# AberHu/TF-NAS

Hardware: AMD Instinct MI355X
Metric: supernet search images/sec (w-step + alpha-step) (higher is better)
Workload: dtype fp32

## Files before the change

tf-nas_amd/csrc/conv_kernels.hip:

```cpp
#include <stdlib.h>
#include "gemm_core.h"
#include "gemm_x3.h"
#include "kernels.h"
#include "prof.h"

constexpr int conv_lb(int mm) { return mm == 0 ? 4 : 3; }
constexpr int conv_wgrad_lb(int nt) { return nt >= 3 ? 3 : 4; }

template <int NT, int MM>
__global__ __launch_bounds__(256, conv_lb(MM)) void k_conv_fwd(TfnasCellDesc d, const float* __restrict__ x,
                                                               float* __restrict__ D, float* __restrict__ part,
                                                               const float* __restrict__ wf) {
    using T = GT<NT>;
    static_assert(T::B_ITERS == 1, "one B item per thread: its K position is the same in every chunk");
    __shared__ __attribute__((aligned(16))) float lds[T::LDS_FLOATS];
    const int BX = blockIdx.x, n0 = blockIdx.y * T::BN;
    const int mc = d.g[0].mc, mcp = d.g[0].mcp, off = d.g[0].off, M = d.M;
    const int H = d.H, W = d.W, Wo = d.Wo, HWo = d.Ho * d.Wo, S = d.stride, ic = d.ic;
    const int Po = d.N * HWo, K = 9 * ic;
    const int nrt = (Po + 127) >> 7, nchunks = (K + 15) >> 4;
    const int tid = threadIdx.x, lane = tid & 63, lr = lane & 15, lk = lane >> 4, wrow = (tid >> 6) * 32;

    float cs[NT], cq[NT];
#pragma unroll
    for (int j = 0; j < NT; ++j) cs[j] = cq[j] = 0.f;

    for (int rt = BX; rt < nrt; rt += gridDim.x) {
        f32x4 acc[2][NT];
        acc_zero<NT>(acc);
        int hi0[2], wi0[2];
        bool rok[2];
        const float* img[2];
#pragma unroll
        for (int i = 0; i < 2; ++i) {
            const int p = rt * 128 + wrow + 16 * i + lr, pc = min(p, Po - 1);
            const int n = pc / HWo, r = pc - n * HWo, ho = r / Wo, wo = r - ho * Wo;
            rok[i] = p < Po;
            hi0[i] = ho * S - 1;
            wi0[i] = wo * S - 1;
            img[i] = x + (size_t)n * H * W * ic;
        }
        int a_ky = 0, a_kx = 0, a_ch = 0;
        bool a_ok = false;
        auto pre = [&](int c) {
            const int ka = c * 16 + 4 * lk;
            a_ok = ka < K;
            const int ta = a_ok ? ka / ic : 0;
            a_ch = a_ok ? ka - ta * ic : 0;
            a_ky = ta / 3;
            a_kx = ta - 3 * a_ky;
        };
        auto tap_ok = [&](int i) -> bool {
            const int hi = hi0[i] + a_ky, wi = wi0[i] + a_kx;
            return a_ok && (unsigned)hi < (unsigned)H && (unsigned)wi < (unsigned)W;
        };
        auto la = [&](int c, int i, int kl) -> f32x4 {
            const int hi = hi0[i] + a_ky, wi = wi0[i] + a_kx;
            const size_t a = tap_ok(i) ? ((size_t)hi * W + wi) * ic + a_ch : 0;
            return ld4(img[i] + a);
        };
        auto xa = [&](f32x4 r, int c, int i, int kl) -> f32x4 { return (rok[i] && tap_ok(i)) ? r : zero4(); };
        auto lb = [&](int c, int n, int kl) -> f32x4 {
            return ld4(wf + (size_t)min(n0 + n, mc - 1) * K + min(c * 16 + kl, K - 4));
        };
        auto xb = [&](f32x4 r, int c, int n, int kl) -> f32x4 { return (c * 16 + kl < K && n0 + n < mc) ? r : zero4(); };
        gemm_adirect<NT, true, MM>(pre, la, xa, lb, xb, nchunks, acc, lds);
        emit_tile_rows<NT>(acc, lds, [&](int lrow, int lc, f32x4 v) {
            const int p = rt * 128 + lrow;
            if (p < Po && n0 + lc < mcp) st4_nt(D + ((size_t)p * M + off + n0 + lc), v);
        });
        acc_colstats<NT>(acc, cs, cq);
    }
    flush_colstats<NT>(cs, cq, lds, part + (size_t)BX * 2 * M + 2 * (size_t)off, n0, mcp);
}

template <int ACT>
__global__ __launch_bounds__(256) void k_conv_dd(TfnasCellDesc d, const float* __restrict__ dZ, const float* __restrict__ D,
                                                 const float* __restrict__ gate, const float* __restrict__ dpooled,
                                                 const double* __restrict__ stats2, const double* __restrict__ red2,
                                                 float* __restrict__ dd) {
    __shared__ f32x4 cst2[64];
    const int mc = d.g[0].mc, mcp = d.g[0].mcp, off = d.g[0].off, M = d.M;
    const int HWo = d.Ho * d.Wo, Po = d.N * HWo, c0 = blockIdx.y * 64;
    const int tid = threadIdx.x, q = tid & 15, ch = c0 + 4 * q;
    fill_cst2(cst2, d, 64, c0, mc, off, stats2, red2);
    __syncthreads();
    if (ch >= mcp) return;
    const bool has_se = d.g[0].se > 0;
    const float inv_hw = 1.f / (float)HWo;
    for (int p = blockIdx.x * 16 + (tid >> 4); p < Po; p += gridDim.x * 16) {
        const size_t a = (size_t)p * M + off + ch;
        const f32x4 dz = ld4_nt(dZ + a), dv = ld4_nt(D + a);
        f32x4 g4 = zero4(), dp4 = zero4();
        if (has_se) {
            const size_t t = (size_t)(p / HWo) * M + off + ch;
            g4 = ld4(gate + t);
            dp4 = ld4(dpooled + t) * splat4(inv_hw);
        }
        f32x4 r = bn2_dd<ACT>(cst2, 4 * q, dz, dv, has_se, g4, dp4);
#pragma unroll
        for (int j = 0; j < 4; ++j)
            if (ch + j >= mc) r[j] = 0.f;
        st4(dd + a, r);
    }
}

struct RawTap { f32x4 v; bool ok; };
template <int NT>
__global__ __launch_bounds__(256, conv_wgrad_lb(NT)) void k_conv_wgrad(TfnasCellDesc d, const float* __restrict__ dd,
                                                                       const float* __restrict__ x, int rows_per_split,
                                                                       float* __restrict__ part, size_t out_size) {
    using T = GT<NT>;
    __shared__ __attribute__((aligned(16))) float lds[T::LDS_FLOATS];
    const int ic = d.ic, mc = d.g[0].mc, mcp = d.g[0].mcp, off = d.g[0].off, M = d.M;
    const int H = d.H, W = d.W, Wo = d.Wo, HWo = d.Ho * d.Wo, S = d.stride, Po = d.N * HWo, NC = 9 * ic;
    float* __restrict__ gw = part + (size_t)blockIdx.x * out_size;
    const int m0 = blockIdx.y * 128, n0 = blockIdx.z * T::BN;
    const int r0 = blockIdx.x * rows_per_split, r1 = min(Po, r0 + rows_per_split);
    const int nchunks = (r1 - r0 + 15) >> 4;
    const int tid = threadIdx.x, lane = tid & 63, lr = lane & 15, lq = lane >> 4, wrow = (tid >> 6) * 32;
// ... 60 lines not shown
    const int W = d.W, HW = d.H * d.W, Ho = d.Ho, Wo = d.Wo, S = d.stride, ic = d.ic;
    const int P = d.N * HW, K = 9 * mcp;
    const int nrt = (P + 127) >> 7, nchunks = (K + 15) >> 4;
    const int tid = threadIdx.x, lane = tid & 63, lr = lane & 15, lk = lane >> 4, wrow = (tid >> 6) * 32;
    constexpr int BQ = T::BN / 4;
    const int bkl = tid / BQ, bcol = n0 + (tid % BQ) * 4;
    const bool bcok = tid < T::B_ITEMS && bcol < ic;
    const int bcc = min(bcol, ic - 4);

    for (int rt = blockIdx.x; rt < nrt; rt += gridDim.x) {
        f32x4 acc[2][NT];
        acc_zero<NT>(acc);
        int hi1[2], wi1[2];
        bool rok[2];
        const float* img[2];
#pragma unroll
        for (int i = 0; i < 2; ++i) {
            const int q = rt * 128 + wrow + 16 * i + lr, qc = min(q, P - 1);
            const int n = qc / HW, r = qc - n * HW, hi = r / W, wi = r - hi * W;
            rok[i] = q < P;
            hi1[i] = hi + 1;
            wi1[i] = wi + 1;
            img[i] = dd + (size_t)n * Ho * Wo * M + off;
        }
        int a_ky = 0, a_kx = 0, a_m = 0;
        bool a_ok = false;
        auto pre = [&](int c) {
            const int ka = c * 16 + 4 * lk;
            a_ok = ka < K;
            const int ta = a_ok ? ka / mcp : 0;
            a_m = a_ok ? ka - ta * mcp : 0;
            a_ky = ta / 3;
            a_kx = ta - 3 * a_ky;
        };
        auto src = [&](int i, int& ho, int& wo) -> bool {
            const int th = hi1[i] - a_ky, tw = wi1[i] - a_kx;
            ho = S == 2 ? th >> 1 : th;
            wo = S == 2 ? tw >> 1 : tw;
            const bool par = S == 1 || !((th | tw) & 1);
            return a_ok && par && th >= 0 && tw >= 0 && ho < Ho && wo < Wo;
        };
        auto la = [&](int c, int i, int kl) -> f32x4 {
            int ho, wo;
            const size_t a = src(i, ho, wo) ? ((size_t)ho * Wo + wo) * M + a_m : 0;
            return ld4(img[i] + a);
        };
        auto xa = [&](f32x4 r, int c, int i, int kl) -> f32x4 {
            int ho, wo;
            return (rok[i] && src(i, ho, wo)) ? r : zero4();
        };
        auto lb = [&](int c, int kl, int n) -> f32x4 { return ld4(wd + (size_t)min(c * 16 + bkl, K - 1) * ic + bcc); };
        auto xb = [&](f32x4 r, int c, int kl, int n) -> f32x4 { return (c * 16 + bkl < K && bcok) ? r : zero4(); };
        gemm_adirect<NT, false, MM>(pre, la, xa, lb, xb, nchunks, acc, lds);
        emit_tile_rows<NT>(acc, lds, [&](int lrow, int lc, f32x4 v) {
            const int q = rt * 128 + lrow;
            if (q < P && n0 + lc < ic) {
                const size_t a = (size_t)q * ic + n0 + lc;
                if (dres) v += ld4_nt(dres + a);
                st4_nt(dx + a, v);
            }
        });
    }
}

__global__ __launch_bounds__(256) void k_conv_repack(TfnasCellDesc d, float* __restrict__ wf, float* __restrict__ wd) {
    const int ic = d.ic, mc = d.g[0].mc, mcp = d.g[0].mcp;
    const float* __restrict__ w = d.g[0].w_expand;
    const int total = (wf ? mc : mcp) * 9 * ic;
    for (int idx = blockIdx.x * 256 + threadIdx.x; idx < total; idx += gridDim.x * 256) {
        if (wf) {
            const int m = idx / (9 * ic), k = idx - m * 9 * ic, tap = k / ic, c = k - tap * ic;
            wf[idx] = w[((size_t)m * ic + c) * 9 + tap];
        } else {
            const int kk = idx / ic, c = idx - kk * ic, tap = kk / mcp, m = kk - tap * mcp;
            wd[idx] = m < mc ? w[((size_t)m * ic + c) * 9 + tap] : 0.f;
        }
    }
}
static size_t conv_repack_floats(const TfnasCellDesc& d) { return ((size_t)9 * d.ic * d.g[0].mcp + 63) & ~(size_t)63; }

#define CONV_MM(mode, ...)                                     \
    switch (mode) {                                            \
        case 0: { constexpr int MM = 0; __VA_ARGS__; } break;  \
        case 1: { constexpr int MM = 1; __VA_ARGS__; } break;  \
        case 3: { constexpr int MM = 3; __VA_ARGS__; } break;  \
        default: { constexpr int MM = 6; __VA_ARGS__; } break; \
    }

static int conv_row_blocks(int rows, int col_tiles, size_t cap, int slots) {
    const int nrt = cdiv(rows, 128);
    int lim = nrt;
    if ((size_t)lim > cap) lim = (int)cap;
    if (lim > 1024) lim = 1024;
    if (lim < 1) lim = 1;
    long best_cost = -1;
    int best = 1;
    for (int gx = 1; gx <= lim; ++gx) {
        const long cost = (long)cdiv(gx * col_tiles, slots) * cdiv(nrt, gx);
        if (best_cost < 0 || cost <= best_cost) {
            best_cost = cost;
            best = gx;
        }
    }
    return best;
}

constexpr size_t CONV_MIN_STAT_ROWS = 128;
// ... 80 lines not shown
```

tf-nas_amd/csrc/gemm_core.h:

```cpp
#pragma once
#include "tfnas_dev.h"

template <int NT>
struct GT {
    static constexpr int BM = 128, BK = 16, BN = 16 * NT;
    static constexpr int LDA = BM + 16;
    static constexpr int LDB = (BN % 32 == 16) ? BN : BN + 16;
    static constexpr int A_FLOATS = BK * LDA, B_FLOATS = BK * LDB;
    static constexpr int X3_FLOATS = 1584 * NT;
    static constexpr int LDS_FLOATS = 2 * (A_FLOATS + B_FLOATS) > X3_FLOATS ? 2 * (A_FLOATS + B_FLOATS) : X3_FLOATS;
    static constexpr int B_ITEMS = BN * 4;
    static constexpr int B_ITERS = (B_ITEMS + 255) / 256;
};

template <int NT>
__device__ __forceinline__ void acc_zero(f32x4 (&acc)[2][NT]) {
#pragma unroll
    for (int i = 0; i < 2; ++i)
#pragma unroll
        for (int j = 0; j < NT; ++j) acc[i][j] = zero4();
}

struct XfId {
    __device__ __forceinline__ f32x4 operator()(f32x4 v, int, int, int, int) const { return v; }
// ... 107 lines not shown
    RB rb[T::B_ITERS];
    f32x4 cur[2];

#define TFNAS_B_IDX(i)                                                      \
    const int idx = tid + 256 * (i), b0_ = BKC ? (idx >> 2) : idx / (T::BN / 4), \
              b1_ = BKC ? (idx & 3) * 4 : (idx % (T::BN / 4)) * 4
#define TFNAS_GLOAD(c)                                                                      \
    {                                                                                       \
        pre(c);                                                                             \
        _Pragma("unroll") for (int i = 0; i < 2; ++i) ra[i] = la((c), i, 4 * lk);           \
        _Pragma("unroll") for (int i = 0; i < T::B_ITERS; ++i) {                            \
            TFNAS_B_IDX(i);                                                                 \
            if (idx < T::B_ITEMS) rb[i] = lb((c), b0_, b1_);                                \
        }                                                                                   \
    }
#define TFNAS_SSTORE(c, Bs)                                                                 \
    {                                                                                       \
        _Pragma("unroll") for (int i = 0; i < 2; ++i) cur[i] = xa(ra[i], (c), i, 4 * lk);   \
        _Pragma("unroll") for (int i = 0; i < T::B_ITERS; ++i) {                            \
            TFNAS_B_IDX(i);                                                                 \
            if (idx < T::B_ITEMS) {                                                         \
                const f32x4 v = xb(rb[i], (c), b0_, b1_);                                   \
                if (BKC) {                          \
                    const int r0_ = b1_ >> 2;                                               \
                    (Bs)[(r0_ + 0) * T::LDB + b0_] = v.x;                                   \
                    (Bs)[(r0_ + 4) * T::LDB + b0_] = v.y;                                   \
                    (Bs)[(r0_ + 8) * T::LDB + b0_] = v.z;                                   \
                    (Bs)[(r0_ + 12) * T::LDB + b0_] = v.w;                                  \
                } else {                                                                    \
                    st4(&(Bs)[((b0_ & 3) * 4 + (b0_ >> 2)) * T::LDB + b1_], v);             \
                }                                                                           \
            }                                                                               \
        }                                                                                   \
    }

    float* Bs0 = lds;
    float* Bs1 = lds + T::B_FLOATS;
    if (nchunks > 0) {
        TFNAS_GLOAD(0);
        TFNAS_SSTORE(0, Bs0);
    }
    __syncthreads();
    for (int c = 0; c < nchunks; ++c) {
        const float* Bs = (c & 1) ? Bs1 : Bs0;
        const bool more = (c + 1 < nchunks);
        if (more) TFNAS_GLOAD(c + 1);
#pragma unroll
        for (int ks = 0; ks < 4; ++ks) {
            const int k = ks * 4 + lk;
            const float a0 = cur[0][ks], a1 = cur[1][ks];
#pragma unroll
            for (int j = 0; j < NT; ++j) {
                const float b = Bs[k * T::LDB + 16 * j + lr];
                acc[0][j] = __builtin_amdgcn_mfma_f32_16x16x4f32(a0, b, acc[0][j], 0, 0, 0);
                acc[1][j] = __builtin_amdgcn_mfma_f32_16x16x4f32(a1, b, acc[1][j], 0, 0, 0);
            }
        }
        if (more) {
            if (c & 1) { TFNAS_SSTORE(c + 1, Bs0); } else { TFNAS_SSTORE(c + 1, Bs1); }
        }
        __syncthreads();
    }
#undef TFNAS_GLOAD
#undef TFNAS_SSTORE
#undef TFNAS_B_IDX
}

template <int NT, bool AK, bool BKC, class FA, class FB>
__device__ __forceinline__ void gemm_mainloop(FA& fa, FB& fb, int nchunks, f32x4 (&acc)[2][NT], float* lds) {
    auto la = [&](int c, int, int i0, int i1) -> f32x4 { return fa(c, i0, i1); };
    auto lb = [&](int c, int, int i0, int i1) -> f32x4 { return fb(c, i0, i1); };
    XfId id;
    gemm_mainloop2<NT, AK, BKC>(la, id, lb, id, nchunks, acc, lds);
}

template <int NT>
__device__ __forceinline__ void acc_colstats(const f32x4 (&acc)[2][NT], float (&s)[NT], float (&q)[NT]) {
#pragma unroll
    for (int j = 0; j < NT; ++j)
#pragma unroll
        for (int i = 0; i < 2; ++i) {
            const f32x4 v = acc[i][j];
            s[j] += (v.x + v.y) + (v.z + v.w);
            q[j] += (v.x * v.x + v.y * v.y) + (v.z * v.z + v.w * v.w);
        }
}

template <int NT>
__device__ __forceinline__ void flush_colstats(float (&s)[NT], float (&q)[NT], float* lds, float* part_row,
                                               int col0, int col_lim) {
    using T = GT<NT>;
    const int tid = threadIdx.x, lane = tid & 63, w = tid >> 6, lr = lane & 15;
#pragma unroll
    for (int j = 0; j < NT; ++j) {
        s[j] += __shfl_xor(s[j], 16, 64);
        s[j] += __shfl_xor(s[j], 32, 64);
        q[j] += __shfl_xor(q[j], 16, 64);
        q[j] += __shfl_xor(q[j], 32, 64);
    }
    if (lane < 16) {
#pragma unroll
        for (int j = 0; j < NT; ++j) {
            lds[(w * 2 + 0) * T::BN + 16 * j + lr] = s[j];
            lds[(w * 2 + 1) * T::BN + 16 * j + lr] = q[j];
        }
    }
    __syncthreads();
    if (tid < T::BN && col0 + tid < col_lim) {
        float ss = 0.f, qq = 0.f;
#pragma unroll
        for (int ww = 0; ww < 4; ++ww) {
            ss += lds[(ww * 2 + 0) * T::BN + tid];
            qq += lds[(ww * 2 + 1) * T::BN + tid];
        }
        part_row[2 * (size_t)(col0 + tid) + 0] = ss;
        part_row[2 * (size_t)(col0 + tid) + 1] = qq;
    }
    __syncthreads();
}

struct SlabNone {
    __device__ __forceinline__ void operator()(int, const float*) const {}
};
template <int NT, class FEmit, class FSlab = SlabNone>
__device__ __forceinline__ void emit_tile_rows(const f32x4 (&acc)[2][NT], float* lds, FEmit emit, FSlab slab = FSlab()) {
    using T = GT<NT>;
    constexpr int LDC = T::BN + 4, Q = T::BN / 4;
    static_assert(4 * 16 * LDC <= T::LDS_FLOATS, "C staging does not fit the GEMM LDS buffer");
    const int tid = threadIdx.x, lane = tid & 63, w = tid >> 6, lr = lane & 15, lq = lane >> 4;
    float* st = lds + w * 16 * LDC;
#pragma unroll
    for (int i = 0; i < 2; ++i) {
        __syncthreads();
#pragma unroll
        for (int j = 0; j < NT; ++j)
#pragma unroll
            for (int r = 0; r < 4; ++r) st[(4 * lq + r) * LDC + 16 * j + lr] = acc[i][j][r];
        __syncthreads();
#pragma unroll
        for (int it = 0; it < (16 * Q + 63) / 64; ++it) {
            const int idx = it * 64 + lane;
            if (idx < 16 * Q) {
                const int row = idx / Q, c4 = idx - row * Q;
                emit(w * 32 + 16 * i + row, 4 * c4, ld4(st + row * LDC + 4 * c4));
            }
        }
        slab(i, st);
    }
    __syncthreads();
}

static inline int pick_nt(int n, const int* cands, int ncand) {
    int best = cands[0];
    long best_pad = -1;
    for (int i = 0; i < ncand; ++i) {
        const int bn = 16 * cands[i];
        const long pad = (long)((n + bn - 1) / bn) * bn;
        if (best_pad < 0 || pad < best_pad || (pad == best_pad && cands[i] > best)) {
            best_pad = pad;
            best = cands[i];
        }
    }
    return best;
}
```

tf-nas_amd/csrc/gemm_kernels.hip:

```cpp
#include <stdlib.h>
#include <string.h>
#include "gemm_core.h"
#include "gemm_x3.h"
#include "kernels.h"
#include "prof.h"

__device__ __forceinline__ f32x4 stem_patch4(const float* __restrict__ img, const TfnasCellDesc& d, int p, int t0) {
    const int HW = d.H * d.W, n = p / HW, r = p - n * HW, ho = r / d.W, wo = r - ho * d.W;
    f32x4 v = zero4();
#pragma unroll
    for (int j = 0; j < 4; ++j) {
        const int t = t0 + j;
        if (t < 27) {
            const int ci = t / 9, rem = t - 9 * ci, ky = rem / 3, kx = rem - 3 * ky;
            const int hi = 2 * ho + ky - 1, wi = 2 * wo + kx - 1;
            if (hi >= 0 && hi < d.Hi && wi >= 0 && wi < d.Wi) v[j] = img[((size_t)(n * 3 + ci) * d.Hi + hi) * d.Wi + wi];
        }
    }
    return v;
}

constexpr int kLbBig = 3, kLbSmall = 4;
constexpr int kLbX3Big = 2, kLbX3Small = 3;
constexpr int gemm_lb(int nt, int mm) { return mm == 0 ? (nt >= 5 ? kLbBig : kLbSmall) : (nt >= 5 ? kLbX3Big : kLbX3Small); }
// ... 6 lines not shown
                                                    float* __restrict__ E, float* __restrict__ part) {
    using T = GT<NT>;
    __shared__ __attribute__((aligned(16))) float lds[T::LDS_FLOATS];
    const int L_ = blockIdx.x + gridDim.x * blockIdx.y;
    const bool ctf_ = d.G > 1;
    const int BX = ctf_ ? L_ / (int)gridDim.y : (int)blockIdx.x;
    int ty = ctf_ ? L_ % (int)gridDim.y : (int)blockIdx.y, g = 0;
    for (; g < d.G - 1; ++g) {
        const int t = (d.g[g].mcp + T::BN - 1) / T::BN;
        if (ty < t) break;
        ty -= t;
    }
    const int mc = d.g[g].mc, mcp = d.g[g].mcp, off = d.g[g].off;
    const float* __restrict__ w = d.g[g].w_expand;
    const int n0 = ty * T::BN;
    const int P = d.N * d.H * d.W, ic = d.ic, M = d.M;
    const int nrt = (P + 127) >> 7, nchunks = (ic + 15) >> 4;
    const int tid = threadIdx.x, lr = tid & 15, wrow = (tid >> 6) * 32;

    float cs[NT], cq[NT];
#pragma unroll
    for (int j = 0; j < NT; ++j) cs[j] = cq[j] = 0.f;

    for (int rt = BX; rt < nrt; rt += gridDim.x) {
        f32x4 acc[2][NT];
        acc_zero<NT>(acc);
        int prow[2];
        const float* arow[2];
#pragma unroll
        for (int i = 0; i < 2; ++i) {
            prow[i] = rt * 128 + wrow + 16 * i + lr;
            arow[i] = x + (size_t)min(prow[i], P - 1) * ic;
        }
        auto la = [&](int c, int i, int kl) -> f32x4 {
            const int k = c * 16 + kl;
            if (STEM) return (prow[i] < P && k < ic) ? stem_patch4(x, d, prow[i], k) : zero4();
            return ld4(arow[i] + min(k, ic - 4));
        };
        auto xa = [&](f32x4 r, int c, int i, int kl) -> f32x4 {
            if (STEM) return r;
            return (prow[i] < P && c * 16 + kl < ic) ? r : zero4();
        };
        auto lb = [&](int c, int n, int kl) -> f32x4 {
            const int col = n0 + n, k = c * 16 + kl;
            if (STEM) return (col < mc) ? ld4_guard(w + (size_t)col * ic, k, ic, false) : zero4();
            return ld4(w + (size_t)min(col, mc - 1) * ic + min(k, ic - 4));
        };
        auto xb = [&](f32x4 r, int c, int n, int kl) -> f32x4 {
            if (STEM) return r;
            return (n0 + n < mc && c * 16 + kl < ic) ? r : zero4();
        };
        PreNone pre;
        gemm_adirect<NT, true, MM>(pre, la, xa, lb, xb, nchunks, acc, lds);
        emit_tile_rows<NT>(acc, lds, [&](int lrow, int lc, f32x4 v) {
            const int p = rt * 128 + lrow;
            if (p < P && n0 + lc < mcp) st4_nt(E + ((size_t)p * M + off + n0 + lc), v);
        });
        acc_colstats<NT>(acc, cs, cq);
    }
    flush_colstats<NT>(cs, cq, lds, part + (size_t)BX * 2 * M + 2 * (size_t)off, n0, mcp);
}

template <int NT, int ACT, int MM>
__global__ __launch_bounds__(256, gemm_lb(NT, MM)) void k_project_fwd(TfnasCellDesc d, const float* __restrict__ D,
                                                     const float* __restrict__ gate,
                                                     const double* __restrict__ stats2, float* __restrict__ Pr,
                                                     float* __restrict__ part, int nsplit, float* __restrict__ prp) {
    using T = GT<NT>;
    extern __shared__ __attribute__((aligned(16))) float lds[];
    const int zr = blockIdx.z / nsplit, ks = blockIdx.z - zr * nsplit;
    int g = 0;
    for (int c = 0; c < d.G; ++c) {
        int rank = 0;
        for (int o = 0; o < d.G; ++o) rank += (d.g[o].mcp > d.g[c].mcp) || (d.g[o].mcp == d.g[c].mcp && o < c);
        if (rank == zr) g = c;
    }
    const int mc = d.g[g].mc, mcp = d.g[g].mcp, off = d.g[g].off;
    const bool has_se = d.g[g].se > 0, w_al = (mc & 3) == 0;
    const float* gbase = has_se ? gate : D;
    const size_t se01 = has_se ? 1 : 0;
    const float* __restrict__ w = d.g[g].w_proj;
    const int n0 = blockIdx.y * T::BN;
    const int HW = d.Ho * d.Wo, Po = d.N * HW, oc = d.oc, M = d.M;
    const int nrt = (Po + 127) >> 7, nchunks_all = (mcp + 15) >> 4;
    const int per = (nchunks_all + nsplit - 1) / nsplit, cb = ks * per;
    const int nchunks = max(0, min(nchunks_all, cb + per) - cb);
    float* __restrict__ dst = ks == 0 ? Pr : prp + (size_t)(ks - 1) * d.G * Po * oc;
    const int tid = threadIdx.x, lr = tid & 15, wrow = (tid >> 6) * 32;

    float2* cst = reinterpret_cast<float2*>(lds + T::LDS_FLOATS);
    for (int c = tid; c < ((mcp + 15) & ~15); c += 256)
        cst[c] = (c < mc) ? bn_consts(stats2 + 2 * (size_t)(off + c), 1.0 / (double)Po, d.eps) : make_float2(0.f, 0.f);
    __syncthreads();

    float cs[NT], cq[NT];
#pragma unroll
    for (int j = 0; j < NT; ++j) cs[j] = cq[j] = 0.f;

    for (int rt = blockIdx.x; rt < nrt; rt += gridDim.x) {
        f32x4 acc[2][NT];
        acc_zero<NT>(acc);
        size_t arow[2], grow[2];
        bool rok[2];
#pragma unroll
        for (int i = 0; i < 2; ++i) {
            const int p = rt * 128 + wrow + 16 * i + lr, pc = min(p, Po - 1);
            rok[i] = p < Po;
            arow[i] = (size_t)pc * M + off;
            grow[i] = ((size_t)(pc / HW) * M + off) * se01;
        }
        auto la = [&](int c, int i, int kl) -> Raw2 {
            const int k = min((cb + c) * 16 + kl, mcp - 4);
            Raw2 r;
            r.a = ld4(D + (arow[i] + k));
            r.b = ld4(gbase + grow[i] + k * se01);
            return r;
        };
        auto xa = [&](Raw2 r, int c, int i, int kl) -> f32x4 {
            const int k = (cb + c) * 16 + kl;
            f32x4 v = r.a;
            const int kc = min(k, mcp - 4);
            const float2 c0 = cst[kc], c1 = cst[kc + 1], c2 = cst[kc + 2], c3 = cst[kc + 3];
            v.x = act_f<ACT>((v.x - c0.x) * c0.y);
            v.y = act_f<ACT>((v.y - c1.x) * c1.y);
            v.z = act_f<ACT>((v.z - c2.x) * c2.y);
            v.w = act_f<ACT>((v.w - c3.x) * c3.y);
            if (has_se) v *= r.b;
            return (rok[i] && k < mcp) ? v : zero4();
        };
        auto lb = [&](int c, int n, int kl) -> f32x4 {
            const int o = n0 + n, k = (cb + c) * 16 + kl;
            if (MM == 0 && !w_al) return (o < oc) ? ld4_guard(w + (size_t)o * mc, k, mc, false) : zero4();
            return ld4(w + (size_t)min(o, oc - 1) * mc + min(k, mc - 4));
        };
        auto xb = [&](f32x4 r, int c, int n, int kl) -> f32x4 {
            if (MM == 0 && !w_al) return r;
            return (n0 + n < oc && (cb + c) * 16 + kl < mc) ? r : zero4();
        };
        PreNone pre;
        gemm_adirect<NT, true, MM>(pre, la, xa, lb, xb, nchunks, acc, lds);
        emit_tile_rows<NT>(acc, lds, [&](int lrow, int lc, f32x4 v) {
            const int p = rt * 128 + lrow;
            if (p < Po && n0 + lc < oc) st4(dst + ((size_t)g * Po + p) * oc + n0 + lc, v);
        });
        acc_colstats<NT>(acc, cs, cq);
    }
    if (nsplit == 1)
        flush_colstats<NT>(cs, cq, lds, part + (size_t)blockIdx.x * 2 * d.G * oc + 2 * (size_t)g * oc, n0, oc);
}

__global__ __launch_bounds__(256) void k_pr_reduce(float* __restrict__ Pr, const float* __restrict__ prp, int nz, int G,
                                                   int Po, int oc, int rps, float* __restrict__ part) {
    __shared__ f32x4 rs[256], rq[256];
    const int tid = threadIdx.x, ocq = oc >> 2, stride = (256 / ocq) * ocq;
    const int g = blockIdx.y;
    const int r0 = blockIdx.x * rps, r1 = min(Po, r0 + rps);
    const size_t base = ((size_t)g * Po + r0) * ocq, zs = (size_t)G * Po * ocq;
    f32x4* __restrict__ p4 = reinterpret_cast<f32x4*>(Pr) + base;
    const f32x4* __restrict__ z4 = reinterpret_cast<const f32x4*>(prp) + base;
    const int n4 = (r1 - r0) * ocq;
    f32x4 s = zero4(), q = zero4();
    if (tid < stride) {
        for (int i = tid; i < n4; i += stride) {
            f32x4 v = p4[i];
            for (int z = 0; z < nz; ++z) v += z4[(size_t)z * zs + i];
            p4[i] = v;
            s += v;
            q += v * v;
        }
    }
    rs[tid] = s;
    rq[tid] = q;
    __syncthreads();
    for (int c = tid; c < oc; c += 256) {
        const int cq = c >> 2, comp = c & 3;
        float ts = 0.f, tq = 0.f;
        for (int k = cq; k < stride; k += ocq) {
            ts += rs[k][comp];
            tq += rq[k][comp];
        }
        float* row = part + (size_t)blockIdx.x * 2 * G * oc + 2 * ((size_t)g * oc + c);
        row[0] = ts;
        row[1] = tq;
    }
}

struct Bn3Tab {
    float *mean, *rstd, *a3, *b3, *c3;
};
__device__ __forceinline__ Bn3Tab bn3_tab_fill(float* base, int ocp, const TfnasCellDesc& d, int g,
                                               const double* stats3, const double* red3, const float* wmix) {
    Bn3Tab t{base, base + ocp, base + 2 * ocp, base + 3 * ocp, base + 4 * ocp};
    const int Po = d.N * d.Ho * d.Wo;
    const double inv = 1.0 / (double)Po;
// ... 125 lines not shown
    constexpr int NC = (T::BN + 63) / 64;
    float2 c2f[NC];
    bool cokf[NC];
    const int HW = d.Ho * d.Wo;
    const bool has_se = d.g[g].se > 0;
    if (FOLD) {
#pragma unroll
        for (int c = 0; c < NC; ++c) {
            const int col = (tid & 63) + 64 * c;
            cokf[c] = col < T::BN && n0 + col < mcp;
            c2f[c] = (cokf[c] && n0 + col < mc) ? bn_consts(stats2 + 2 * (size_t)(off + n0 + col), 1.0 / (double)Po, d.eps)
                                               : make_float2(0.f, 0.f);
        }
    }
    __syncthreads();

    for (int rt = BX; rt < nrt; rt += gridDim.x) {
        f32x4 acc[2][NT];
        acc_zero<NT>(acc);
        const float* drow[2];
        const float* qrow[2];
        bool rok[2];
#pragma unroll
        for (int i = 0; i < 2; ++i) {
            const int p = rt * 128 + wrow + 16 * i + lr, pc = min(p, Po - 1);
            rok[i] = p < Po;
            drow[i] = dout + (size_t)pc * oc;
            qrow[i] = Pr + ((size_t)g * Po + pc) * oc;
        }
        auto la = [&](int c, int i, int kl) -> Raw2 {
            const int o = min(c * 16 + kl, oc - 4);
            Raw2 r;
            r.a = ld4(drow[i] + o);
            r.b = ld4(qrow[i] + o);
            return r;
        };
        auto xa = [&](Raw2 r, int c, int i, int kl) -> f32x4 {
            const int o = c * 16 + kl;
            const f32x4 v = bn3_fold_dp(tab, min(o, oc - 4), r.a, r.b);
            return (rok[i] && o < oc) ? v : zero4();
        };
        auto lb = [&](int c, int kl, int n) -> f32x4 {
            const int o = c * 16 + kl;
            if (MM == 0 && !w_al) return (o < oc) ? ld4_guard(w + (size_t)o * mc, n0 + n, mc, false) : zero4();
            return ld4(w + (size_t)min(o, oc - 1) * mc + min(n0 + n, mc - 4));
        };
        auto xb = [&](f32x4 r, int c, int kl, int n) -> f32x4 {
            if (MM == 0 && !w_al) return r;
            return (c * 16 + kl < oc && n0 + n < mc) ? r : zero4();
        };
        PreNone pre;
        gemm_adirect<NT, false, MM>(pre, la, xa, lb, xb, nchunks, acc, lds);
        if (!FOLD) {
            emit_tile_rows<NT>(acc, lds, [&](int lrow, int lc, f32x4 v) {
                const int p = rt * 128 + lrow;
                if (p < Po && n0 + lc < mcp) st4_nt(dZ + ((size_t)p * M + off + n0 + lc), v);
            });
        } else {
            constexpr int LDC = T::BN + 4;
            const int w = tid >> 6, lane = tid & 63;
            const int pw0 = rt * 128 + w * 32;
            const int imgA = min(pw0, Po - 1) / HW, bnd = (imgA + 1) * HW;
            float sum[2][FOLD_Q][NC];
#pragma unroll
            for (int a = 0; a < 2; ++a)
#pragma unroll
                for (int q = 0; q < FOLD_Q; ++q)
#pragma unroll
                    for (int c = 0; c < NC; ++c) sum[a][q][c] = 0.f;
            const float* Dcol = D + off + n0;
            emit_tile_rows<NT>(acc, lds,
                               [&](int lrow, int lc, f32x4 v) {
                                   const int p = rt * 128 + lrow;
                                   if (p < Po && n0 + lc < mcp) st4_nt(dZ + ((size_t)p * M + off + n0 + lc), v);
                               },
                               [&](int i, const float* st) {
                                   if (d.act == TFNAS_ACT_RELU)
                                       fold_slab<NT, TFNAS_ACT_RELU>(st, LDC, Dcol, M, pw0 + 16 * i, Po, bnd, c2f, cokf, has_se, sum);
                                   else
                                       fold_slab<NT, TFNAS_ACT_SWISH>(st, LDC, Dcol, M, pw0 + 16 * i, Po, bnd, c2f, cokf, has_se, sum);
                               });
            static_assert(4 * 2 * FOLD_Q * T::BN + 4 <= T::LDS_FLOATS, "fold staging does not fit the GEMM LDS buffer");
            float* comb = lds;
            int* meta = reinterpret_cast<int*>(lds + 4 * 2 * FOLD_Q * T::BN);
#pragma unroll
            for (int a = 0; a < 2; ++a)
#pragma unroll
                for (int q = 0; q < FOLD_Q; ++q)
#pragma unroll
                    for (int c = 0; c < NC; ++c)
                        if (lane + 64 * c < T::BN) comb[((w * 2 + a) * FOLD_Q + q) * T::BN + lane + 64 * c] = sum[a][q][c];
            if (lane == 0) meta[w] = imgA;
            __syncthreads();
            const int img0 = min(rt * 128, Po - 1) / HW, imgL = min(rt * 128 + 127, Po - 1) / HW;
            const int nq = has_se ? FOLD_Q : 2;
            for (int o = tid; o < FOLD_SLOTS * FOLD_Q * T::BN; o += 256) {
                const int sl = o / (FOLD_Q * T::BN), q = (o / T::BN) % FOLD_Q, col = o % T::BN;
                if (img0 + sl > imgL || q >= nq || n0 + col >= mcp) continue;
                float t = 0.f;
#pragma unroll
                for (int ww = 0; ww < 4; ++ww)
#pragma unroll
                    for (int a = 0; a < 2; ++a)
                        if (meta[ww] + a - img0 == sl) t += comb[((ww * 2 + a) * FOLD_Q + q) * T::BN + col];
                rec[(((size_t)rt * FOLD_SLOTS + sl) * FOLD_Q + q) * M + off + n0 + col] = t;
            }
            __syncthreads();
        }
    }
}

constexpr int wgrad_lb(int nt) { return nt >= 5 ? 2 : (nt >= 3 ? 3 : 4); }

template <int NT, int ACT>
__global__ __launch_bounds__(256, wgrad_lb(NT)) void k_project_wgrad(TfnasCellDesc d, const float* __restrict__ dout,
                                                       const float* __restrict__ Pr, const float* __restrict__ D,
                                                       const float* __restrict__ gate,
                                                       const double* __restrict__ stats2,
                                                       const double* __restrict__ stats3,
                                                       const double* __restrict__ red3,
                                                       const float* __restrict__ wmix, int rows_per_split,
                                                       int ntiles_o, float* __restrict__ part, size_t out_size) {
    using T = GT<NT>;
    extern __shared__ __attribute__((aligned(16))) float lds[];
    const int g = blockIdx.z / ntiles_o, n0 = (blockIdx.z % ntiles_o) * T::BN;
    const int mc = d.g[g].mc, mcp = d.g[g].mcp, off = d.g[g].off;
    const bool has_se = d.g[g].se > 0;
    const float* gbase = has_se ? gate : D;
    const size_t se01 = has_se ? 1 : 0;
    size_t poff = 0;
    for (int gg = 0; gg < g; ++gg) poff += (size_t)d.g[gg].mc * d.oc;
    float* __restrict__ gw = part + (size_t)blockIdx.x * out_size + poff;
    const int m0 = blockIdx.y * 128;
    if (m0 >= mcp) return;
// ... 148 lines not shown
        bool is_x;
        int k0, klim_a, klim_b, ld_a;
        size_t aoff;
        const float* bsrc;
        const float* ssrc;
        auto pre = [&](int c) {
            c += cbeg;
            if (c >= mchunks) {
                is_x = true;
                k0 = (c - mchunks) * 16;
                klim_a = klim_b = ld_a = ic;
                aoff = 0;
                bsrc = gram;
                ssrc = cb1 + 1;
                return;
            }
            int g = 0;
            for (; g < d.G - 1; ++g) {
                const int t = (d.g[g].mcp + 15) >> 4;
                if (c < t) break;
                c -= t;
            }
            is_x = false;
            k0 = c * 16;
            klim_a = d.g[g].mcp;
            klim_b = d.g[g].mc;
            ld_a = M;
            aoff = d.g[g].off;
            bsrc = d.g[g].w_expand;
            ssrc = cb1 + 4 * (size_t)d.g[g].off + 1;
        };
        int prow[2];
#pragma unroll
        for (int i = 0; i < 2; ++i) prow[i] = rt * 128 + wrow + 16 * i + lr;
        auto la = [&](int c, int i, int kl) -> f32x4 {
            const int pc = min(prow[i], P - 1), k = min(k0 + kl, klim_a - 4);
            return ld4((is_x ? x : dEh) + (size_t)pc * ld_a + aoff + k);
        };
        auto xa = [&](f32x4 r, int c, int i, int kl) -> f32x4 {
            return (prow[i] < P && k0 + kl < klim_a) ? r : zero4();
        };
        auto lb = [&](int c, int kl, int n) -> RawWS {
            const int kc = min(k0 + kl, klim_b - 1), col = min(n0 + n, ic - 4);
            RawWS r;
            r.w = ld4(bsrc + (size_t)kc * ic + col);
            r.s = ssrc[is_x ? 0 : 4 * (size_t)kc];
            return r;
        };
        auto xb = [&](RawWS r, int c, int kl, int n) -> f32x4 {
            const f32x4 v = is_x ? -r.w : splat4(r.s) * r.w;
            return (n0 + n < ic && k0 + kl < klim_b) ? v : zero4();
        };
        gemm_adirect<NT, false, MM>(pre, la, xa, lb, xb, nchunks, acc, lds);
        emit_tile_rows<NT>(acc, lds, [&](int lrow, int lc, f32x4 v) {
            const int p = rt * 128 + lrow, c = n0 + lc;
            if (p < P && c < ic) {
                if (plain) v += ld4(gram + (size_t)ic * ic + c);
                if (add_res) v += splat4(sumw) * ld4(dout + (size_t)p * d.oc + c);
                if (add_sink) v = sink_add(v, sink_w, ld4(add_src + (size_t)p * ic + c));
                st4(dst + (size_t)p * ic + c, v);
            }
        });
    }
}

__global__ __launch_bounds__(256) void k_dx_reduce(TfnasCellDesc d, const float* __restrict__ dxp, int nsplit,
                                                   const float* __restrict__ gram, const float* __restrict__ dout,
                                                   const float* __restrict__ wmix, float* __restrict__ dx,
                                                   const float* __restrict__ add_src,
                                                   const float* __restrict__ add_scale) {
    const float sink_w = add_src ? add_scale[0] : 0.f;
    const size_t n4 = (size_t)d.N * d.H * d.W * d.ic / 4;
    const int iq = d.ic / 4;
    const float* __restrict__ bias = gram + (size_t)d.ic * d.ic;
    float sumw = 1.f;
    if (wmix) {
        sumw = 0.f;
        for (int g = 0; g < d.G; ++g) sumw += wmix[g];
    }
    for (size_t i = (size_t)blockIdx.x * 256 + threadIdx.x; i < n4; i += (size_t)gridDim.x * 256) {
        f32x4 v = ld4(bias + 4 * (int)(i % iq));
        if (d.has_res) v += splat4(sumw) * ld4(dout + 4 * i);
        for (int z = 0; z < nsplit; ++z) v += ld4(dxp + (size_t)z * n4 * 4 + 4 * i);
        if (add_src) v = sink_add(v, sink_w, ld4(add_src + 4 * i));
        st4(dx + 4 * i, v);
    }
}

template <int NT>
__global__ __launch_bounds__(256) void k_expand_gram(TfnasCellDesc d, const float* __restrict__ cb1, int chunks_per_split,
                                                     int nsplit, float* __restrict__ part) {
    using T = GT<NT>;
    __shared__ __attribute__((aligned(16))) float lds[T::LDS_FLOATS];
    const int ic = d.ic;
    const int m0 = blockIdx.y * 128, n0 = blockIdx.z * T::BN;
    const int xs = (int)blockIdx.x;
    int mchunks = 0;
    for (int g = 0; g < d.G; ++g) mchunks += (d.g[g].mcp + 15) >> 4;
    const int cbeg = xs * chunks_per_split;
    const int nchunks = max(0, min(mchunks, cbeg + chunks_per_split) - cbeg);
    const f32x4* cb = reinterpret_cast<const f32x4*>(cb1);
    const int tid = threadIdx.x, lane = tid & 63, lr = lane & 15, lq = lane >> 4, wrow = (tid >> 6) * 32;
    float* __restrict__ out = part + (size_t)blockIdx.x * (size_t)(ic + 4) * ic;

    f32x4 acc[2][NT];
    acc_zero<NT>(acc);
    auto locate = [&](int c, int& g, int& k0) {
// ... 628 lines not shown
```

tf-nas_amd/csrc/gemm_x3.h:

```cpp
#pragma once
#include "gemm_core.h"

typedef __bf16 bf16x8 __attribute__((ext_vector_type(8)));
typedef unsigned u32x4 __attribute__((ext_vector_type(4)));
typedef unsigned u32x2 __attribute__((ext_vector_type(2)));

__device__ __forceinline__ unsigned x3_bits(float v) { return __builtin_bit_cast(unsigned, v); }
__device__ __forceinline__ float x3_float(unsigned v) { return __builtin_bit_cast(float, v); }
__device__ __forceinline__ unsigned x3_pack(unsigned a, unsigned b) { return __builtin_amdgcn_perm(b, a, 0x07060302u); }

struct X3Planes { u32x2 h, m, l; };
template <int TERMS>
__device__ __forceinline__ X3Planes x3_split4(f32x4 v) {
    unsigned hb[4], mb[4], lb[4];
#pragma unroll
    for (int e = 0; e < 4; ++e) {
        hb[e] = x3_bits(v[e]);
        mb[e] = lb[e] = 0;
        if (TERMS > 1) {
            const float r1 = v[e] - x3_float(hb[e] & 0xffff0000u);
            mb[e] = x3_bits(r1);
            if (TERMS > 3) lb[e] = x3_bits(r1 - x3_float(mb[e] & 0xffff0000u));
        }
    }
// ... 63 lines not shown
                                         : (b1 >> 4) * X::TS + (4 * h + (b0 >> 2)) * 128 + (b0 & 3) * 32 + ((b1 & 15) >> 2) * 8;
                *reinterpret_cast<u32x2*>(Bs + off) = p.h;
                if (TERMS > 1) *reinterpret_cast<u32x2*>(Bs + PLANE + off) = p.m;
                if (TERMS > 3) *reinterpret_cast<u32x2*>(Bs + 2 * PLANE + off) = p.l;
            }
        }
    };
    auto sstore = [&](int C, unsigned char* Bs) {
        X3Planes p0[2], p1[2];
        sstore_half(2 * C, 0, true, Bs, p0);
        sstore_half(2 * C + 1, 1, 2 * C + 1 < nchunks, Bs, p1);
#pragma unroll
        for (int i = 0; i < 2; ++i) {
            ca[i][0] = u32x4{p0[i].h.x, p0[i].h.y, p1[i].h.x, p1[i].h.y};
            ca[i][1] = u32x4{p0[i].m.x, p0[i].m.y, p1[i].m.x, p1[i].m.y};
            ca[i][2] = u32x4{p0[i].l.x, p0[i].l.y, p1[i].l.x, p1[i].l.y};
        }
    };
    const unsigned rd = BKC ? lr * 64 + ((lk ^ x3_fperm(lr >> 2)) * 16) : lk * 128 + lr * 8;
    auto frag = [&](const unsigned char* p, int j) -> bf16x8 {
        if (BKC) return __builtin_bit_cast(bf16x8, *reinterpret_cast<const u32x4*>(p + rd + j * 1024));
        typedef short s16x4 __attribute__((ext_vector_type(4)));
        typedef short s16x8 __attribute__((ext_vector_type(8)));
        typedef __attribute__((address_space(3))) s16x4* lds_p;
        const s16x4 a = __builtin_amdgcn_ds_read_tr16_b64_v4i16((lds_p)(p + rd + j * X::TS));
        const s16x4 b = __builtin_amdgcn_ds_read_tr16_b64_v4i16((lds_p)(p + rd + j * X::TS + 512));
        const s16x8 v = {a.x, a.y, a.z, a.w, b.x, b.y, b.z, b.w};
        return __builtin_bit_cast(bf16x8, v);
    };

    if (nC > 0) {
        gload(0);
        sstore(0, lds);
    }
    __syncthreads();
    for (int C = 0; C < nC; ++C) {
        const unsigned char* Bs = lds + (C & 1) * BUF;
        const bool more = C + 1 < nC;
        if (more) gload(C + 1);
        bf16x8 ah[2], am[2], al[2];
#pragma unroll
        for (int i = 0; i < 2; ++i) {
            ah[i] = __builtin_bit_cast(bf16x8, ca[i][0]);
            am[i] = __builtin_bit_cast(bf16x8, ca[i][1]);
            al[i] = __builtin_bit_cast(bf16x8, ca[i][2]);
        }
#pragma unroll
        for (int j = 0; j < NT; ++j) {
            const bf16x8 bh = frag(Bs, j);
            bf16x8 bm = bh, bl = bh;
            if (TERMS > 1) bm = frag(Bs + PLANE, j);
            if (TERMS > 3) bl = frag(Bs + 2 * PLANE, j);
#define TFNAS_X3_MF(a, b)                                                                   \
    acc[0][j] = __builtin_amdgcn_mfma_f32_16x16x32_bf16(a[0], b, acc[0][j], 0, 0, 0);       \
    acc[1][j] = __builtin_amdgcn_mfma_f32_16x16x32_bf16(a[1], b, acc[1][j], 0, 0, 0);
            if (TERMS > 3) { TFNAS_X3_MF(al, bh) TFNAS_X3_MF(am, bm) TFNAS_X3_MF(ah, bl) }
            if (TERMS > 1) { TFNAS_X3_MF(am, bh) TFNAS_X3_MF(ah, bm) }
            TFNAS_X3_MF(ah, bh)
#undef TFNAS_X3_MF
        }
        if (more) sstore(C + 1, lds + ((C + 1) & 1) * BUF);
        __syncthreads();
    }
}

template <int NT, bool BKC, int MM, class PRE, class LA, class XA, class LB, class XB>
__device__ __forceinline__ void gemm_adirect(PRE& pre, LA& la, XA& xa, LB& lb, XB& xb, int nchunks, f32x4 (&acc)[2][NT],
                                             float* lds) {
    if constexpr (MM == 0) gemm_mainloop_adirect<NT, BKC>(pre, la, xa, lb, xb, nchunks, acc, lds);
    else gemm_mainloop_adirect_x3<NT, BKC, MM>(pre, la, xa, lb, xb, nchunks, acc, lds);
}
```

Before: 3908.

## Swap MFMA operands to transpose accumulator layout and simplify epilogues

Swaps the A/B operands of the MFMA instructions so each lane holds four consecutive output columns of one row instead of four rows of one column. With this transposed accumulator layout, several GEMM epilogues store f32x4 results straight to global memory without LDS staging. The remaining staged paths use per-wave vector LDS writes with wave-level ordering instead of block-wide barriers, and column statistics are reduced with DPP row operations instead of cross-lane shuffles. This removes LDS round-trips and __syncthreads in the epilogue, but relies on the new lane-to-element mapping being applied consistently everywhere acc is consumed.

Measured after the change: 3882 (median of 2 runs). About the same (-0.6%).

```diff
diff --git a/tf-nas_amd/csrc/conv_kernels.hip b/tf-nas_amd/csrc/conv_kernels.hip
--- a/tf-nas_amd/csrc/conv_kernels.hip
+++ b/tf-nas_amd/csrc/conv_kernels.hip
@@ -65,7 +65,7 @@
         };
         auto xb = [&](f32x4 r, int c, int n, int kl) -> f32x4 { return (c * 16 + kl < K && n0 + n < mc) ? r : zero4(); };
         gemm_adirect<NT, true, MM>(pre, la, xa, lb, xb, nchunks, acc, lds);
-        emit_tile_rows<NT>(acc, lds, [&](int lrow, int lc, f32x4 v) {
+        emit_tile_staged<NT>(acc, lds, [&](int lrow, int lc, f32x4 v) {
             const int p = rt * 128 + lrow;
             if (p < Po && n0 + lc < mcp) st4_nt(D + ((size_t)p * M + off + n0 + lc), v);
         });
@@ -232,7 +232,7 @@
         auto lb = [&](int c, int kl, int n) -> f32x4 { return ld4(wd + (size_t)min(c * 16 + bkl, K - 1) * ic + bcc); };
         auto xb = [&](f32x4 r, int c, int kl, int n) -> f32x4 { return (c * 16 + bkl < K && bcok) ? r : zero4(); };
         gemm_adirect<NT, false, MM>(pre, la, xa, lb, xb, nchunks, acc, lds);
-        emit_tile_rows<NT>(acc, lds, [&](int lrow, int lc, f32x4 v) {
+        emit_tile_direct<NT>(acc, [&](int lrow, int lc, f32x4 v) {
             const int q = rt * 128 + lrow;
             if (q < P && n0 + lc < ic) {
                 const size_t a = (size_t)q * ic + n0 + lc;
diff --git a/tf-nas_amd/csrc/gemm_core.h b/tf-nas_amd/csrc/gemm_core.h
--- a/tf-nas_amd/csrc/gemm_core.h
+++ b/tf-nas_amd/csrc/gemm_core.h
@@ -183,8 +183,8 @@
 #pragma unroll
             for (int j = 0; j < NT; ++j) {
                 const float b = Bs[k * T::LDB + 16 * j + lr];
-                acc[0][j] = __builtin_amdgcn_mfma_f32_16x16x4f32(a0, b, acc[0][j], 0, 0, 0);
-                acc[1][j] = __builtin_amdgcn_mfma_f32_16x16x4f32(a1, b, acc[1][j], 0, 0, 0);
+                acc[0][j] = __builtin_amdgcn_mfma_f32_16x16x4f32(b, a0, acc[0][j], 0, 0, 0);
+                acc[1][j] = __builtin_amdgcn_mfma_f32_16x16x4f32(b, a1, acc[1][j], 0, 0, 0);
             }
         }
         if (more) {
@@ -205,35 +205,44 @@
     gemm_mainloop2<NT, AK, BKC>(la, id, lb, id, nchunks, acc, lds);
 }
 
+template <int CTRL>
+__device__ __forceinline__ float dpp_mov(float v) {
+    return __builtin_bit_cast(float, __builtin_amdgcn_update_dpp(0, __builtin_bit_cast(int, v), CTRL, 0xf, 0xf, false));
+}
+__device__ __forceinline__ float rows16_sum(f32x4 v, bool hi, bool odd) {
+    const float x = v.x + dpp_mov<0x140>(v.x), y = v.y + dpp_mov<0x140>(v.y);
+    const float z = v.z + dpp_mov<0x140>(v.z), w = v.w + dpp_mov<0x140>(v.w);
+    float k0 = hi ? z : x, k1 = hi ? w : y;
+    k0 += dpp_mov<0x141>(k0);
+    k1 += dpp_mov<0x141>(k1);
+    float m = odd ? k1 : k0;
+    m += dpp_mov<0xB1>(m);
+    m += dpp_mov<0x4E>(m);
+    return m;
+}
+
 template <int NT>
 __device__ __forceinline__ void acc_colstats(const f32x4 (&acc)[2][NT], float (&s)[NT], float (&q)[NT]) {
-#pragma unroll
-    for (int j = 0; j < NT; ++j)
-#pragma unroll
-        for (int i = 0; i < 2; ++i) {
-            const f32x4 v = acc[i][j];
-            s[j] += (v.x + v.y) + (v.z + v.w);
-            q[j] += (v.x * v.x + v.y * v.y) + (v.z * v.z + v.w * v.w);
-        }
+    const int lr = threadIdx.x & 15;
+    const bool hi = (lr & 8) != 0, odd = (lr & 4) != 0;
+#pragma unroll
+    for (int j = 0; j < NT; ++j) {
+        const f32x4 a = acc[0][j], b = acc[1][j];
+        s[j] += rows16_sum(a + b, hi, odd);
+        q[j] += rows16_sum(a * a + b * b, hi, odd);
+    }
 }
 
 template <int NT>
 __device__ __forceinline__ void flush_colstats(float (&s)[NT], float (&q)[NT], float* lds, float* part_row,
                                                int col0, int col_lim) {
     using T = GT<NT>;
-    const int tid = threadIdx.x, lane = tid & 63, w = tid >> 6, lr = lane & 15;
-#pragma unroll
-    for (int j = 0; j < NT; ++j) {
-        s[j] += __shfl_xor(s[j], 16, 64);
-        s[j] += __shfl_xor(s[j], 32, 64);
-        q[j] += __shfl_xor(q[j], 16, 64);
-        q[j] += __shfl_xor(q[j], 32, 64);
-    }
-    if (lane < 16) {
+    const int tid = threadIdx.x, lane = tid & 63, w = tid >> 6, lr = lane & 15, lq = lane >> 4;
+    if ((lr & 3) == 0) {
 #pragma unroll
         for (int j = 0; j < NT; ++j) {
-            lds[(w * 2 + 0) * T::BN + 16 * j + lr] = s[j];
-            lds[(w * 2 + 1) * T::BN + 16 * j + lr] = q[j];
+            lds[(w * 2 + 0) * T::BN + 16 * j + 4 * lq + (lr >> 2)] = s[j];
+            lds[(w * 2 + 1) * T::BN + 16 * j + 4 * lq + (lr >> 2)] = q[j];
         }
     }
     __syncthreads();
@@ -248,26 +257,45 @@
         part_row[2 * (size_t)(col0 + tid) + 1] = qq;
     }
     __syncthreads();
+}
+
+template <int NT, class FEmit>
+__device__ __forceinline__ void emit_tile_direct(const f32x4 (&acc)[2][NT], FEmit emit) {
+    const int tid = threadIdx.x, lane = tid & 63, w = tid >> 6, lr = lane & 15, lq = lane >> 4;
+#pragma unroll
+    for (int i = 0; i < 2; ++i)
+#pragma unroll
+        for (int j = 0; j < NT; ++j) emit(w * 32 + 16 * i + lr, 16 * j + 4 * lq, acc[i][j]);
+}
+
+__device__ __forceinline__ void wave_lds_order() {
+    asm volatile("s_waitcnt lgkmcnt(0)" ::: "memory");
+    __builtin_amdgcn_wave_barrier();
+}
+template <int NT>
+__device__ __forceinline__ float* stage_slab_wave(const f32x4 (&acc)[2][NT], int i, float* lds) {
+    using T = GT<NT>;
+    constexpr int LDC = T::BN + 4;
+    static_assert(4 * 16 * LDC <= T::LDS_FLOATS, "C staging does not fit the GEMM LDS buffer");
+    const int tid = threadIdx.x, lane = tid & 63, w = tid >> 6, lr = lane & 15, lq = lane >> 4;
+    float* st = lds + w * 16 * LDC;
+#pragma unroll
+    for (int j = 0; j < NT; ++j) st4(st + lr * LDC + 16 * j + 4 * lq, acc[i][j]);
+    return st;
 }
 
 struct SlabNone {
     __device__ __forceinline__ void operator()(int, const float*) const {}
 };
 template <int NT, class FEmit, class FSlab = SlabNone>
-__device__ __forceinline__ void emit_tile_rows(const f32x4 (&acc)[2][NT], float* lds, FEmit emit, FSlab slab = FSlab()) {
+__device__ __forceinline__ void emit_tile_staged(const f32x4 (&acc)[2][NT], float* lds, FEmit emit, FSlab slab = FSlab()) {
     using T = GT<NT>;
     constexpr int LDC = T::BN + 4, Q = T::BN / 4;
-    static_assert(4 * 16 * LDC <= T::LDS_FLOATS, "C staging does not fit the GEMM LDS buffer");
-    const int tid = threadIdx.x, lane = tid & 63, w = tid >> 6, lr = lane & 15, lq = lane >> 4;
-    float* st = lds + w * 16 * LDC;
+    const int tid = threadIdx.x, lane = tid & 63, w = tid >> 6;
 #pragma unroll
     for (int i = 0; i < 2; ++i) {
-        __syncthreads();
-#pragma unroll
-        for (int j = 0; j < NT; ++j)
-#pragma unroll
-            for (int r = 0; r < 4; ++r) st[(4 * lq + r) * LDC + 16 * j + lr] = acc[i][j][r];
-        __syncthreads();
+        const float* st = stage_slab_wave<NT>(acc, i, lds);
+        wave_lds_order();
 #pragma unroll
         for (int it = 0; it < (16 * Q + 63) / 64; ++it) {
             const int idx = it * 64 + lane;
@@ -277,6 +305,7 @@
             }
         }
         slab(i, st);
+        wave_lds_order();
     }
     __syncthreads();
 }
diff --git a/tf-nas_amd/csrc/gemm_kernels.hip b/tf-nas_amd/csrc/gemm_kernels.hip
--- a/tf-nas_amd/csrc/gemm_kernels.hip
+++ b/tf-nas_amd/csrc/gemm_kernels.hip
@@ -82,10 +82,12 @@
         };
         PreNone pre;
         gemm_adirect<NT, true, MM>(pre, la, xa, lb, xb, nchunks, acc, lds);
-        emit_tile_rows<NT>(acc, lds, [&](int lrow, int lc, f32x4 v) {
+        auto emit = [&](int lrow, int lc, f32x4 v) {
             const int p = rt * 128 + lrow;
             if (p < P && n0 + lc < mcp) st4_nt(E + ((size_t)p * M + off + n0 + lc), v);
-        });
+        };
+        if constexpr (STEM) emit_tile_direct<NT>(acc, emit);
+        else emit_tile_staged<NT>(acc, lds, emit);
         acc_colstats<NT>(acc, cs, cq);
     }
     flush_colstats<NT>(cs, cq, lds, part + (size_t)BX * 2 * M + 2 * (size_t)off, n0, mcp);
@@ -169,7 +171,7 @@
         };
         PreNone pre;
         gemm_adirect<NT, true, MM>(pre, la, xa, lb, xb, nchunks, acc, lds);
-        emit_tile_rows<NT>(acc, lds, [&](int lrow, int lc, f32x4 v) {
+        emit_tile_direct<NT>(acc, [&](int lrow, int lc, f32x4 v) {
             const int p = rt * 128 + lrow;
             if (p < Po && n0 + lc < oc) st4(dst + ((size_t)g * Po + p) * oc + n0 + lc, v);
         });
@@ -401,7 +403,7 @@
         PreNone pre;
         gemm_adirect<NT, false, MM>(pre, la, xa, lb, xb, nchunks, acc, lds);
         if (!FOLD) {
-            emit_tile_rows<NT>(acc, lds, [&](int lrow, int lc, f32x4 v) {
+            emit_tile_staged<NT>(acc, lds, [&](int lrow, int lc, f32x4 v) {
                 const int p = rt * 128 + lrow;
                 if (p < Po && n0 + lc < mcp) st4_nt(dZ + ((size_t)p * M + off + n0 + lc), v);
             });
@@ -418,17 +420,17 @@
 #pragma unroll
                     for (int c = 0; c < NC; ++c) sum[a][q][c] = 0.f;
             const float* Dcol = D + off + n0;
-            emit_tile_rows<NT>(acc, lds,
-                               [&](int lrow, int lc, f32x4 v) {
-                                   const int p = rt * 128 + lrow;
-                                   if (p < Po && n0 + lc < mcp) st4_nt(dZ + ((size_t)p * M + off + n0 + lc), v);
-                               },
-                               [&](int i, const float* st) {
-                                   if (d.act == TFNAS_ACT_RELU)
-                                       fold_slab<NT, TFNAS_ACT_RELU>(st, LDC, Dcol, M, pw0 + 16 * i, Po, bnd, c2f, cokf, has_se, sum);
-                                   else
-                                       fold_slab<NT, TFNAS_ACT_SWISH>(st, LDC, Dcol, M, pw0 + 16 * i, Po, bnd, c2f, cokf, has_se, sum);
-                               });
+            emit_tile_staged<NT>(acc, lds,
+                                 [&](int lrow, int lc, f32x4 v) {
+                                     const int p = rt * 128 + lrow;
+                                     if (p < Po && n0 + lc < mcp) st4_nt(dZ + ((size_t)p * M + off + n0 + lc), v);
+                                 },
+                                 [&](int i, const float* st) {
+                                     if (d.act == TFNAS_ACT_RELU)
+                                         fold_slab<NT, TFNAS_ACT_RELU>(st, LDC, Dcol, M, pw0 + 16 * i, Po, bnd, c2f, cokf, has_se, sum);
+                                     else
+                                         fold_slab<NT, TFNAS_ACT_SWISH>(st, LDC, Dcol, M, pw0 + 16 * i, Po, bnd, c2f, cokf, has_se, sum);
+                                 });
             static_assert(4 * 2 * FOLD_Q * T::BN + 4 <= T::LDS_FLOATS, "fold staging does not fit the GEMM LDS buffer");
             float* comb = lds;
             int* meta = reinterpret_cast<int*>(lds + 4 * 2 * FOLD_Q * T::BN);
@@ -683,7 +685,7 @@
             return (n0 + n < ic && k0 + kl < klim_b) ? v : zero4();
         };
         gemm_adirect<NT, false, MM>(pre, la, xa, lb, xb, nchunks, acc, lds);
-        emit_tile_rows<NT>(acc, lds, [&](int lrow, int lc, f32x4 v) {
+        emit_tile_direct<NT>(acc, [&](int lrow, int lc, f32x4 v) {
             const int p = rt * 128 + lrow, c = n0 + lc;
             if (p < P && c < ic) {
                 if (plain) v += ld4(gram + (size_t)ic * ic + c);
diff --git a/tf-nas_amd/csrc/gemm_x3.h b/tf-nas_amd/csrc/gemm_x3.h
--- a/tf-nas_amd/csrc/gemm_x3.h
+++ b/tf-nas_amd/csrc/gemm_x3.h
@@ -139,8 +139,8 @@
             if (TERMS > 1) bm = frag(Bs + PLANE, j);
             if (TERMS > 3) bl = frag(Bs + 2 * PLANE, j);
 #define TFNAS_X3_MF(a, b)                                                                   \
-    acc[0][j] = __builtin_amdgcn_mfma_f32_16x16x32_bf16(a[0], b, acc[0][j], 0, 0, 0);       \
-    acc[1][j] = __builtin_amdgcn_mfma_f32_16x16x32_bf16(a[1], b, acc[1][j], 0, 0, 0);
+    acc[0][j] = __builtin_amdgcn_mfma_f32_16x16x32_bf16(b, a[0], acc[0][j], 0, 0, 0);       \
+    acc[1][j] = __builtin_amdgcn_mfma_f32_16x16x32_bf16(b, a[1], acc[1][j], 0, 0, 0);
             if (TERMS > 3) { TFNAS_X3_MF(al, bh) TFNAS_X3_MF(am, bm) TFNAS_X3_MF(ah, bl) }
             if (TERMS > 1) { TFNAS_X3_MF(am, bh) TFNAS_X3_MF(ah, bm) }
             TFNAS_X3_MF(ah, bh)
```
